# tooHotSpot/FGN

Measured on AMD Instinct MI355X. Metric: query-imgs/sec (3-way 3-shot, 800x1333 FGN simple_test), higher is better.
Workload: dtype f32; 1 GPU; cfg3: COCO2VOC 3-way 3-shot, query 3x800x1333, supports 9x3x256^2, ResNet-50-C4, R<=300 proposals, D<=100 detections, 1 episode(s) per GPU per step; h2d_in_step=True, gt_mask_rle_in_step=True, world_size_seen=1, phase_lock=rpn, caller_streams=2, support_cache=False, hip_graph=True, winograd_3x3=F(4x4,3x3)

## Files before the change

fgn_amd/csrc/conv_igemm.hip:

```cpp
#include "common.h"
#include <cstdlib>

struct ConvParams {
    const float* x;
    const float* w;
    float* y;
    const float* scale;
    const float* shift;
    const float* residual;
    const float* in_scale;
    const int32_t* n_img_dev;
    int n_img, H, W, Cin, Ho, Wo, Cout, KH, KW, stride, pad;
    int a_img_div;
    int relu;
    int K;
    int n_tiles_n;
    int band_nt, band_mt;
    float* ws;
    int splits, kt_per_split;
#ifdef FGN_EXPERIMENTS
    int32_t* tickets;
    int32_t* sched;
    int sk_U, sk_dp;
#endif
// ... 1378 lines not shown
                                            const void* w_x3, float* y, const float* shift, int rows, int Cin1, int Cin2,
                                            int Cout, int cout_pad, int relu, hipStream_t stream) {
    if (!x || !x2 || !w_x3 || !y) return FGN_ERR_ARG;
    if (rows <= 0) return FGN_OK;
    if (Cin1 % BK || Cin2 % BK || Cin1 <= 0 || Cin2 <= 0 || (Cout & 3) || cout_pad % X3_BN || cout_pad < Cout) return FGN_ERR_SHAPE;
    if ((!x2_rows && x2_total_rows != rows) || x2_total_rows < 1) return FGN_ERR_ARG;
    const int K = Cin1 + Cin2;
    const long long xb = (long long)rows * Cin1 * 4, x2b = (long long)x2_total_rows * Cin2 * 4;
    const long long wb = (long long)fgn_x3_image_bytes(K, cout_pad, 1);
    if (xb >= 0x7fffff00ll || x2b >= 0x7fffff00ll || wb >= 0x7fffff00ll || (long long)rows * Cout >= (1ll << 31)) return FGN_ERR_SHAPE;
    ConvParams p;
    x3_base_params(p);
    p.x = x; p.y = y; p.shift = shift;
    p.x2 = x2; p.x2_bytes = (unsigned)x2b; p.kt1 = Cin1 / BK; p.cin2 = Cin2; p.x2_rows = x2_rows;
    p.n_img = rows; p.Cin = Cin1; p.Cout = Cout; p.relu = relu; p.K = K;
    p.kt_per_split = K / BK; p.x_bytes = (unsigned)xb;
    p.w3 = w_x3; p.w3_bytes = (unsigned)wb; p.npad3 = cout_pad;
    return launch_x3(p, rows, 0, 6, stream);
}

extern "C" int fgn_winograd_gemm_x3_f32(const float* V, const void* U_x3, float* Mo, const int32_t* n_img_dev, int n_img,
                                        int tiles_per_img, int t_pad, int Cin, int Cout, int cout_pad, int n_groups,
                                        hipStream_t stream) {
    if (!V || !U_x3 || !Mo) return FGN_ERR_ARG;
    if (n_img <= 0) return FGN_OK;
    if (Cin % BK != 0 || Cin < 2 * BK || Cout % 4 != 0 || cout_pad % X3_BN != 0 || cout_pad < Cout || t_pad % 64 != 0 ||
        (n_groups != 16 && n_groups != 36) || (long long)n_img * tiles_per_img > t_pad)
        return FGN_ERR_SHAPE;
    const long long rows = (long long)n_groups * t_pad;
    const long long xb = rows * Cin * 4, wb = (long long)fgn_x3_image_bytes(Cin, cout_pad, n_groups);
    if (xb >= 0x7fffff00ll || wb >= 0x7fffff00ll || rows * Cout >= (1ll << 31)) return FGN_ERR_SHAPE;
    ConvParams p;
    x3_base_params(p);
    p.x = V; p.y = Mo;
    p.n_img = (int)rows; p.Cin = Cin; p.Cout = Cout; p.K = Cin; p.kt_per_split = Cin / BK; p.x_bytes = (unsigned)xb;
    p.grp_rows = t_pad; p.grp_valid = n_img * tiles_per_img; p.grp_items = n_img;
    p.grp_rows_per_item = tiles_per_img; p.grp_count_dev = n_img_dev;
    p.w3 = U_x3; p.w3_bytes = (unsigned)wb; p.npad3 = cout_pad;
    return launch_x3(p, (int)rows, 0, 6, stream);
}

static int h2_pick(long long M, int Cout, int K, int grp_rows, int grp_valid, int bm) {
    if (bm == 264) return (grp_rows && grp_rows % 128) ? 0 : 264;
    if (bm != 0) return x3_pick_bm(M, Cout, K, grp_rows, grp_valid, bm);
    if (Cout <= 64) {
        if (grp_rows && grp_rows % 128) return 0;
        if (Cout < 48 || (M + 127) / 128 < 256) return 0;
        return 264;
    }
    const int bm_x3 = x3_pick_bm(M, Cout, K, grp_rows, grp_valid, 0);
    return (bm_x3 == 128 && !grp_rows) ? 64 : bm_x3;
}

template <int WMW, int WNW, int RB, int NST, bool IM2COL>
static int launch_h2_cfg(ConvParams& p, const H2Im2col& q2, int M_max, hipStream_t stream) {
    constexpr int BM = 32 * RB * WMW, BN = 64 * WNW;
    const int m_tiles = cdiv(M_max, BM);
    p.n_tiles_n = cdiv(p.Cout, BN);
    {
        const long long per_nt = (long long)BN * p.K * 4;
        p.band_nt = 0; p.band_mt = 0;
        if (per_nt * p.n_tiles_n > 2048 * 1024) {
            int nb = (int)std::max<long long>(1, 2048 * 1024 / per_nt);
            while (nb > 1 && p.n_tiles_n % nb) --nb;
            const int mt = p.grp_rows ? p.grp_rows / BM : m_tiles;
            if (nb < p.n_tiles_n && mt > 0 && m_tiles % mt == 0) { p.band_nt = nb; p.band_mt = mt; }
        }
    }
    const int tiles = m_tiles * p.n_tiles_n;
    static unsigned long long ok = 0ull;
    hipError_t attr = fgn_allow_full_lds(reinterpret_cast<const void*>(conv_pw_h2_kernel<WMW, WNW, RB, NST, IM2COL>), &ok);
    if (attr != hipSuccess) return (int)attr;
    const size_t lds = (size_t)NST * (BM * 128 + 2 * BN * 64);
    const int per_cu = std::min(3, (int)(160 * 1024 / lds));
    const int grid = std::min(256 * per_cu, (tiles + 7) / 8 * 8);
    p.stamp = fgn_next_stamp_record();
    FGN_LAUNCH_TIMED((conv_pw_h2_kernel<WMW, WNW, RB, NST, IM2COL>), dim3(grid), dim3(64 * WMW * WNW), lds, stream, p, q2, tiles);
    FGN_LAUNCH_CHECK();
    return FGN_OK;
}

extern "C" size_t fgn_h2_image_bytes(int K, int npad, int n_groups) { return (size_t)n_groups * npad * ((size_t)K * 4 + 4); }
extern "C" int fgn_h2_row_tile(long long M, int Cout, int K, int grp_rows, int grp_valid) {
    return h2_pick(M, Cout, K, grp_rows, grp_valid, 0);
}

static int launch_h2(const ConvParams& p0, int M_max, int n_groups, int bm, hipStream_t stream, const H2Im2col* im = nullptr) {
    ConvParams p = p0;
    if (!p.w3 || p.npad3 % H2_BN || p.npad3 < p.Cout || (p.Cout & 3) || p.K % BK || p.K < 2 * BK || p.splits != 1) return FGN_ERR_SHAPE;
    const size_t img = (size_t)n_groups * p.K * p.npad3 * 4;
    p.w3_bytes = (unsigned)img;
    p.w_inv = reinterpret_cast<const float*>(static_cast<const char*>(p.w3) + img);
    H2Im2col none;
    none.y1 = nullptr; none.x_off0 = none.x_off1 = 0u; none.M0 = none.M1 = 0; none.H1 = none.W1 = none.Ho1 = none.Wo1 = 1; none.cin_shift = 0;
    if (bm != 0 && bm != 64 && bm != 128 && bm != 264) return FGN_ERR_SHAPE;
    const int cfg = h2_pick(M_max, p.Cout, p.K, p.grp_rows, p.grp_valid, bm);
    if (cfg == 0) return FGN_ERR_SHAPE;
    if (im) {
        if (cfg == 264) return launch_h2_cfg<4, 1, 1, 2, true>(p, *im, M_max, stream);
        return cfg == 128 ? launch_h2_cfg<2, 2, 2, 2, true>(p, *im, M_max, stream) : launch_h2_cfg<2, 2, 1, 2, true>(p, *im, M_max, stream);
    }
    if (cfg == 264) return launch_h2_cfg<4, 1, 1, 2, false>(p, none, M_max, stream);
    return cfg == 128 ? launch_h2_cfg<2, 2, 2, 2, false>(p, none, M_max, stream) : launch_h2_cfg<2, 2, 1, 2, false>(p, none, M_max, stream);
}

extern "C" int fgn_conv2d_pair_h2_nhwc_f32(const float* x0, int n_img0, int H0, int W0, const float* x1, int n_img1, int H1,
                                           int W1, const void* w_h2, float* y0, float* y1, const float* scale,
                                           const float* shift, int Cin, int Cout, int cout_pad, int KH, int KW, int stride,
                                           int pad, int relu, hipStream_t stream) {
    if (!x0 || !w_h2 || !y0 || (x1 && !y1)) return FGN_ERR_ARG;
    if (n_img0 <= 0 || (x1 && n_img1 <= 0)) return FGN_ERR_SHAPE;
    const int ct = Cin / BK;
    if (Cin % BK || (ct & (ct - 1)) || KH != KW || (KW != 1 && KW != 3) || stride < 1 || pad < 0 || (Cout & 3) ||
        cout_pad % H2_BN || cout_pad < Cout || H0 <= 0 || W0 <= 0)
        return FGN_ERR_SHAPE;
    const int Ho0 = (H0 + 2 * pad - KH) / stride + 1, Wo0 = (W0 + 2 * pad - KW) / stride + 1;
    const int Ho1 = x1 ? (H1 + 2 * pad - KH) / stride + 1 : 1, Wo1 = x1 ? (W1 + 2 * pad - KW) / stride + 1 : 1;
    if (Ho0 <= 0 || Wo0 <= 0 || Ho1 <= 0 || Wo1 <= 0) return FGN_ERR_SHAPE;
    const long long M0 = (long long)n_img0 * Ho0 * Wo0, M1 = x1 ? (long long)n_img1 * Ho1 * Wo1 : 0;
    const long long b0 = (long long)n_img0 * H0 * W0 * Cin * 4, b1 = x1 ? (long long)n_img1 * H1 * W1 * Cin * 4 : 0;
    const char* lo = reinterpret_cast<const char*>(x0);
    if (x1 && reinterpret_cast<const char*>(x1) < lo) lo = reinterpret_cast<const char*>(x1);
    const long long off0 = reinterpret_cast<const char*>(x0) - lo, off1 = x1 ? reinterpret_cast<const char*>(x1) - lo : 0;
    const long long span = std::max(off0 + b0, off1 + b1);
    const int K = KH * KW * Cin;
    const long long wb = (long long)fgn_h2_image_bytes(K, cout_pad, 1);
    if (span >= 0x7fffff00ll || wb >= 0x7fffff00ll || (M0 + M1) * Cout >= (1ll << 31)) return FGN_ERR_SHAPE;
    ConvParams p;
    x3_base_params(p);
    p.x = reinterpret_cast<const float*>(lo); p.x_bytes = (unsigned)span; p.y = y0; p.scale = scale; p.shift = shift;
    p.n_img = n_img0; p.H = H0; p.W = W0; p.Ho = Ho0; p.Wo = Wo0; p.Cin = Cin; p.Cout = Cout; p.relu = relu;
    p.KH = KH; p.KW = KW; p.stride = stride; p.pad = pad; p.K = K; p.kt_per_split = K / BK;
    p.w3 = w_h2; p.npad3 = cout_pad;
    H2Im2col q;
    q.y1 = y1; q.x_off0 = (unsigned)off0; q.x_off1 = (unsigned)off1; q.M0 = (int)M0; q.M1 = (int)M1;
    q.H1 = x1 ? H1 : 1; q.W1 = x1 ? W1 : 1; q.Ho1 = Ho1; q.Wo1 = Wo1;
    q.cin_shift = 0;
    while ((1 << q.cin_shift) < ct) ++q.cin_shift;
    return launch_h2(p, (int)(M0 + M1), 1, 0, stream, &q);
}

extern "C" int fgn_gemm_h2_f32(const float* x, const void* w_h2, float* y, const float* shift, const float* residual,
                               int rows, int K, int Cout, int npad, int relu, int grp_rows, int grp_valid, int n_groups,
                               int bm, hipStream_t stream) {
    if (!x || !w_h2 || !y) return FGN_ERR_ARG;
    if (rows <= 0) return FGN_OK;
    if (K % BK || K <= 0 || (Cout & 3) || npad % H2_BN || npad < Cout || n_groups < 1) return FGN_ERR_SHAPE;
    if (n_groups > 1 && (grp_rows <= 0 || (long long)n_groups * grp_rows != rows || grp_valid > grp_rows)) return FGN_ERR_SHAPE;
    const long long xb = (long long)rows * K * 4, wb = (long long)fgn_h2_image_bytes(K, npad, n_groups);
    if (xb >= 0x7fffff00ll || wb >= 0x7fffff00ll || (long long)rows * Cout >= (1ll << 31)) return FGN_ERR_SHAPE;
    ConvParams p;
    x3_base_params(p);
    p.x = x; p.y = y; p.shift = shift; p.residual = residual;
    p.n_img = rows; p.Cin = K; p.Cout = Cout; p.relu = relu; p.K = K; p.kt_per_split = K / BK; p.x_bytes = (unsigned)xb;
    p.grp_rows = n_groups > 1 ? grp_rows : 0; p.grp_valid = grp_valid;
    p.w3 = w_h2; p.npad3 = npad;
// ... 98 lines not shown
```

fgn_amd/csrc/conv_pw_h2.h:

```cpp
#pragma once

typedef _Float16 f16x8_t __attribute__((ext_vector_type(8)));

struct H2Frag { f16x8_t hi, lo; };

__device__ __forceinline__ void h2_split4(const float x0, const float x1, const float x2, const float x3, const float s,
                                          unsigned& h01, unsigned& h23, unsigned& l01, unsigned& l23) {
    asm("v_fma_mixlo_f16 %0, %4, %8, 0\n\t"
        "v_fma_mixlo_f16 %1, %6, %8, 0\n\t"
        "v_fma_mixhi_f16 %0, %5, %8, 0\n\t"
        "v_fma_mixhi_f16 %1, %7, %8, 0\n\t"
        "v_fma_mixlo_f16 %2, %4, %8, -%0 op_sel:[0,0,0] op_sel_hi:[0,0,1]\n\t"
        "v_fma_mixlo_f16 %3, %6, %8, -%1 op_sel:[0,0,0] op_sel_hi:[0,0,1]\n\t"
        "v_fma_mixhi_f16 %2, %5, %8, -%0 op_sel:[0,0,1] op_sel_hi:[0,0,1]\n\t"
        "v_fma_mixhi_f16 %3, %7, %8, -%1 op_sel:[0,0,1] op_sel_hi:[0,0,1]\n\t"
        "s_nop 1"
        : "=&v"(h01), "=&v"(h23), "=&v"(l01), "=&v"(l23)
        : "v"(x0), "v"(x1), "v"(x2), "v"(x3), "s"(s));
}

__device__ __forceinline__ H2Frag h2_split(const float4& a, const float4& b, const float s) {
    unsigned h[4], l[4];
    h2_split4(a.x, a.y, a.z, a.w, s, h[0], h[1], l[0], l[1]);
    h2_split4(b.x, b.y, b.z, b.w, s, h[2], h[3], l[2], l[3]);
    H2Frag f;
    f.hi = __builtin_bit_cast(f16x8_t, make_uint4(h[0], h[1], h[2], h[3]));
    f.lo = __builtin_bit_cast(f16x8_t, make_uint4(l[0], l[1], l[2], l[3]));
    return f;
}

__device__ __forceinline__ float h2_absmax16(const float4& a, const float4& b, const float4& c, const float4& d) {
    float m;
    asm("v_max3_f32 %0, |%1|, |%2|, 0\n\t"
        "v_max3_f32 %0, |%3|, |%4|, %0\n\t"
        "v_max3_f32 %0, |%5|, |%6|, %0\n\t"
        "v_max3_f32 %0, |%7|, |%8|, %0\n\t"
        "v_max3_f32 %0, |%9|, |%10|, %0\n\t"
        "v_max3_f32 %0, |%11|, |%12|, %0\n\t"
        "v_max3_f32 %0, |%13|, |%14|, %0\n\t"
        "v_max3_f32 %0, |%15|, |%16|, %0"
        : "=&v"(m)
        : "v"(a.x), "v"(a.y), "v"(a.z), "v"(a.w), "v"(b.x), "v"(b.y), "v"(b.z), "v"(b.w),
          "v"(c.x), "v"(c.y), "v"(c.z), "v"(c.w), "v"(d.x), "v"(d.y), "v"(d.z), "v"(d.w));
    return m;
}

constexpr int H2_BN = 128;

struct H2Im2col {
    float* y1;
    unsigned x_off0, x_off1;
    int M0, M1;
    int H1, W1, Ho1, Wo1;
    int cin_shift;
};

template <int WMW, int WNW, int RB, int NST, bool IM2COL>
__global__ __launch_bounds__(64 * WMW * WNW, 2) void conv_pw_h2_kernel(const ConvParams p, const H2Im2col q2, const int total_tiles) {
    constexpr int BM = 32 * RB * WMW, BN = 64 * WNW, NTHR = 64 * WMW * WNW, NW = WMW * WNW;
    constexpr int A_LD = BM / 8 / NW;
    constexpr int A_STAGE = BM * 128;
    constexpr int B_STAGE = 2 * BN * 64;
    constexpr int STAGE = A_STAGE + B_STAGE;
    constexpr int BQ = BN / 16;
    constexpr int B_LD = 2 * BQ / NW;
    static_assert(A_LD * 8 * NW == BM && B_LD * NW == 2 * BQ, "tile / wave split");
    constexpr int PER = A_LD + B_LD;
    constexpr int D = NST - 1;
    constexpr int ROWS_PER_PASS = NTHR / 8;
    static_assert(NST == 2 || NST == 3, "ring of 2 or 3 stages");
    extern __shared__ __attribute__((aligned(16))) unsigned char smem_h2[];

    const int t = threadIdx.x, lane = t & 63, wv = t >> 6;
    const int wm = wv / WNW, wn = wv % WNW;
    const int M = IM2COL ? q2.M0 + q2.M1 : (p.n_img_dev ? min(p.n_img, *p.n_img_dev) : p.n_img) * p.Ho * p.Wo;
    int grp_valid = p.grp_valid;
    if (p.grp_rows && p.grp_count_dev) grp_valid = min(grp_valid, min(p.grp_items, *p.grp_count_dev) * p.grp_rows_per_item);

    float a_s = 1.f, a_inv = 1.f;

    const int col4 = t & 7, row0 = t >> 3;
    const int src_c4 = col4 ^ ((row0 >> 1) & 7);
    const i32x4 x_rs = make_rsrc(p.x, p.x_bytes);
    const i32x4 w_rs = make_rsrc(p.w3, p.w3_bytes);
    const bool dual = !IM2COL && p.x2 != nullptr;
    const i32x4 x2_rs = make_rsrc(dual ? p.x2 : p.x, dual ? p.x2_bytes : p.x_bytes);
    const int KT = p.K / BK;
    const unsigned kt_bytes = (unsigned)(2 * p.npad3 * 64);
    const unsigned lds_base = __builtin_amdgcn_readfirstlane((unsigned)reinterpret_cast<size_t>(smem_h2));
    const unsigned wave_row_bytes = __builtin_amdgcn_readfirstlane(wv) * 8 * 128;
    constexpr unsigned OOB = 0x7ffffff0u;

    const int nq = total_tiles >> 3, nr = total_tiles & 7;
    auto coords = [&](int tile, int& m0, int& n0) -> bool {
        const int xcd = tile & 7, idx = tile >> 3;
        const int bid = (xcd < nr ? xcd * (nq + 1) : nr * (nq + 1) + (xcd - nr) * nq) + idx;
        int tile_m = bid / p.n_tiles_n;
        int tile_n = bid - tile_m * p.n_tiles_n;
        if (p.band_nt > 0) {
            const int per_grp = p.band_mt * p.n_tiles_n;
            const int grp = bid / per_grp;
            int r = bid - grp * per_grp;
            const int per_band = p.band_mt * p.band_nt;
            const int band = r / per_band;
            r -= band * per_band;
            const int mi = r / p.band_nt;
            tile_m = grp * p.band_mt + mi;
            tile_n = band * p.band_nt + (r - mi * p.band_nt);
        }
        m0 = tile_m * BM;
        n0 = tile_n * BN;
        if (m0 >= M) return false;
// ... 39 lines not shown
                        for (int kx = 0; kx < p.KW; ++kx, ++tp)
                            if (y_ok && (unsigned)(ix0 + kx) < (unsigned)W) tm |= 1u << tp;
                    }
                    o.a2[i] = tm;
                }
                continue;
            }
            const bool in = m < M && m < g_end;
            o.a[i] = in ? (unsigned)((m * p.Cin + src_c4 * 4) * 4) : OOB;
            o.a2[i] = OOB;
            if (dual && in) o.a2[i] = (unsigned)(((p.x2_rows ? p.x2_rows[m] : m) * p.cin2 + src_c4 * 4) * 4);
        }
        unsigned g0 = 0;
        if (p.grp_rows) g0 = (unsigned)(m0 / p.grp_rows) * (unsigned)KT * kt_bytes;
#pragma unroll
        for (int i = 0; i < B_LD; ++i) {
            const int q = wv + NW * i;
            const int plane = q / BQ, row = (q % BQ) * 16 + (lane >> 2);
            o.b[i] = g0 + (unsigned)(((plane * p.npad3 + n0 + row) * 4 + (lane & 3)) * 16);
        }
        return o;
    };
    auto issue = [&](const Offs& o, int kt, int stage) {
        const unsigned st = lds_base + stage * STAGE;
        const unsigned sa = st + wave_row_bytes;
        const unsigned ko = (unsigned)(kt * BK * 4);
        if constexpr (IM2COL) {
            const int tap = kt >> q2.cin_shift;
            const int c0 = (kt - (tap << q2.cin_shift)) * BK;
            const int ky = p.KW == 3 ? (tap * 43) >> 7 : tap;
            const int kx = tap - ky * p.KW;
            const unsigned off0 = (unsigned)(((ky * p.W + kx) * p.Cin + c0) * 4);
            const unsigned off1 = (unsigned)(((ky * q2.W1 + kx) * p.Cin + c0) * 4);
#pragma unroll
            for (int i = 0; i < A_LD; ++i) {
                const bool ok = (o.a2[i] >> tap) & 1u;
                const unsigned voff = ok ? o.a[i] + ((o.a2[i] >> 31) ? off1 : off0) : OOB;
                lds_dma16_s(x_rs, sa + i * ROWS_PER_PASS * 128, voff, 0u);
            }
        } else if (dual && kt >= p.kt1) {
            const unsigned ko2 = (unsigned)((kt - p.kt1) * BK * 4);
#pragma unroll
            for (int i = 0; i < A_LD; ++i) lds_dma16_s(x2_rs, sa + i * ROWS_PER_PASS * 128, o.a2[i], ko2);
        } else {
#pragma unroll
            for (int i = 0; i < A_LD; ++i) lds_dma16_s(x_rs, sa + i * ROWS_PER_PASS * 128, o.a[i], ko);
        }
        const unsigned kb = (unsigned)kt * kt_bytes;
#pragma unroll
        for (int i = 0; i < B_LD; ++i) lds_dma16_s(w_rs, st + b_lds[i], o.b[i], kb);
    };

    const int r16 = lane & 15, g4 = lane >> 4;
    const int a16_row = wm * 32 * RB + r16;
    const unsigned a16_sw = (unsigned)((a16_row >> 1) & 7);
    const unsigned a16_rd0 = (unsigned)(a16_row * 128) + ((((unsigned)g4) ^ a16_sw) << 4);
    const unsigned a16_rd1 = (unsigned)(a16_row * 128) + ((((unsigned)(g4 + 4)) ^ a16_sw) << 4);
    const int n16 = wn * 64 + r16;
    const unsigned tau16 = (0x1230u >> (4 * ((n16 >> 2) & 3))) & 3u;
    const unsigned b16_rd = (unsigned)(A_STAGE + n16 * 64) + ((((unsigned)g4) ^ tau16) << 4);

    if (p.stamp && t == 0 && blockIdx.x == 0) atomicExch(p.stamp, __builtin_amdgcn_s_memrealtime());
    auto leave = [&]() {
        if (!p.stamp || t != 0) return;
        const unsigned shard = blockIdx.x & 7u;
        const unsigned long long in_shard = (gridDim.x - shard + 7u) / 8u;
        unsigned long long* const sc = p.stamp + 8 * (1 + shard);
        if (atomicAdd(sc, 1ull) != in_shard - 1) return;
        atomicExch(sc, 0ull);
        const unsigned long long shards = gridDim.x < 8u ? gridDim.x : 8u;
        if (atomicAdd(p.stamp + 2, 1ull) != shards - 1) return;
        const unsigned long long d = __builtin_amdgcn_s_memrealtime() - atomicExch(p.stamp, 0ull);
        atomicExch(p.stamp + 2, 0ull);
        atomicAdd(p.stamp + 1, d);
        atomicAdd(p.stamp + 3, 1ull);
        atomicMin(p.stamp + 4, d);
        atomicMax(p.stamp + 5, d);
    };

    int m0, n0, nm0 = 0, nn0 = 0;
    int tile = next_active(blockIdx.x, m0, n0);
    if (tile < 0) { leave(); return; }
    Offs cur = offsets(m0, n0);
    int ntile = next_active(tile + gridDim.x, nm0, nn0);
    Offs nxt = cur;
    if (ntile >= 0) nxt = offsets(nm0, nn0);
    int ic_kt = 0, ic_stage = 0, ahead = 0;
    bool ic_next = false;
    auto issue_one = [&]() {
        if (!ic_next) {
            issue(cur, ic_kt, ic_stage);
            if (++ic_kt == KT) { ic_next = true; ic_kt = 0; }
        } else {
            if (ntile < 0 || ic_kt >= KT) return;
            issue(nxt, ic_kt, ic_stage);
            ++ic_kt;
        }
        ic_stage = ic_stage + 1 == NST ? 0 : ic_stage + 1;
        ++ahead;
    };
#pragma unroll
    for (int i = 0; i < D; ++i) issue_one();
    int stage = 0;

    while (true) {
        f32x4 acc[2 * RB][4];
#pragma unroll
        for (int i = 0; i < 2 * RB; ++i)
#pragma unroll
            for (int j = 0; j < 4; ++j) acc[i][j] = f32x4{0.f, 0.f, 0.f, 0.f};
        bool have_s = false;
        float a_lim = 0.f;
        a_s = 1.f; a_inv = 1.f;
        for (int kt = 0; kt < KT; ++kt) {
            if (D == 2 && kt > 0 && ahead == 2) x3_wait_vm<PER>(); else x3_wait_vm<0>();
            asm volatile("s_waitcnt lgkmcnt(0)" ::: "memory");
            __builtin_amdgcn_s_barrier();
            --ahead;
            issue_one();
            asm volatile("" ::: "memory");
            const unsigned char* const S = smem_h2 + stage * STAGE;
            float4 alo[2 * RB], ahi[2 * RB];
            f16x8_t bq[4][2];
#pragma unroll
            for (int i = 0; i < 2 * RB; ++i) {
                alo[i] = *reinterpret_cast<const float4*>(S + a16_rd0 + i * (16 * 128));
                ahi[i] = *reinterpret_cast<const float4*>(S + a16_rd1 + i * (16 * 128));
            }
#pragma unroll
            for (int j = 0; j < 4; ++j)
#pragma unroll
                for (int q = 0; q < 2; ++q)
                    bq[j][q] = *reinterpret_cast<const f16x8_t*>(S + b16_rd + j * (16 * 64) + q * (BN * 64));
            __builtin_amdgcn_sched_barrier(0);
            auto adapt = [&]() {
                float m = 0.f;
#pragma unroll
                for (int i = 0; i < 2 * RB; ++i) {
                    m = fmaxf(m, fmaxf(fmaxf(fabsf(alo[i].x), fabsf(alo[i].y)), fmaxf(fabsf(alo[i].z), fabsf(alo[i].w))));
                    m = fmaxf(m, fmaxf(fmaxf(fabsf(ahi[i].x), fabsf(ahi[i].y)), fmaxf(fabsf(ahi[i].z), fabsf(ahi[i].w))));
                }
#pragma unroll
                for (int o = 32; o > 0; o >>= 1) m = fmaxf(m, __shfl_xor(m, o));
                const unsigned mb = __builtin_amdgcn_readfirstlane(__float_as_uint(m));
                const int e = (int)((mb >> 23) & 0xffu);
                if (e < 27 || e == 255) return;
                const float ns = __uint_as_float((unsigned)(267 - e) << 23);
                const float ratio = ns * a_inv;
                if (have_s) {
#pragma unroll
                    for (int i = 0; i < 2 * RB; ++i)
#pragma unroll
                        for (int j = 0; j < 4; ++j) acc[i][j] *= ratio;
                }
                a_s = ns;
                a_inv = __uint_as_float((unsigned)(e - 13) << 23);
                a_lim = 65504.f * a_inv;
                have_s = true;
            };
            {
                float big = h2_absmax16(alo[0], ahi[0], alo[1], ahi[1]);
                if constexpr (RB == 2) big = fmaxf(big, h2_absmax16(alo[2], ahi[2], alo[3], ahi[3]));
                if (__builtin_expect(__builtin_amdgcn_ballot_w64(!(big <= a_lim)) != 0ull, 0)) adapt();
            }
#pragma unroll
            for (int i = 0; i < 2 * RB; ++i) {
                const H2Frag a = h2_split(alo[i], ahi[i], a_s);
#pragma unroll
                for (int j = 0; j < 4; ++j) {
                    f32x4 c = acc[i][j];
                    c = __builtin_amdgcn_mfma_f32_16x16x32_f16(a.lo, bq[j][0], c, 0, 0, 0);
                    c = __builtin_amdgcn_mfma_f32_16x16x32_f16(a.hi, bq[j][1], c, 0, 0, 0);
                    c = __builtin_amdgcn_mfma_f32_16x16x32_f16(a.hi, bq[j][0], c, 0, 0, 0);
                    acc[i][j] = c;
                }
            }
            stage = stage + 1 == NST ? 0 : stage + 1;
        }
        float* const cbase = reinterpret_cast<float*>(smem_h2 + (stage == 0 ? NST - 1 : stage - 1) * STAGE);
        const int em0 = m0, en0 = n0;
        const float* const winv = p.w_inv + (p.grp_rows ? (size_t)(em0 / p.grp_rows) * p.npad3 : 0);
        constexpr int PR = 32 * RB;
#pragma unroll
        for (int pass = 0; pass < WMW; ++pass) {
            __syncthreads();
            if (wm == pass) {
#pragma unroll
                for (int i = 0; i < 2 * RB; ++i)
#pragma unroll
                    for (int j = 0; j < 4; ++j) {
                        float* cw = cbase + (16 * i + 4 * g4) * BN + wn * 64 + 16 * j + r16;
#pragma unroll
                        for (int r = 0; r < 4; ++r) cw[r * BN] = acc[i][j][r] * a_inv;
                    }
            }
            __syncthreads();
            constexpr int C4 = BN / 4, RPP = NTHR / C4, NPASS = PR / RPP, SW = NPASS < 4 ? NPASS : 4;
            static_assert(NPASS % SW == 0, "row sweeps in groups of SW");
            const int c4 = t % C4, rr = t / C4;
            const int n = en0 + c4 * 4;
            if (n < p.Cout) {
                float4 sc = make_float4(1.f, 1.f, 1.f, 1.f), sh = make_float4(0.f, 0.f, 0.f, 0.f);
                if (p.scale) sc = *reinterpret_cast<const float4*>(p.scale + n);
                if (p.shift) sh = *reinterpret_cast<const float4*>(p.shift + n);
                const float4 iv = *reinterpret_cast<const float4*>(winv + n);
#pragma unroll
                for (int k0 = 0; k0 < NPASS; k0 += SW) {
                    float4 res[SW];
#pragma unroll
                    for (int k = 0; k < SW; ++k) {
                        const int m = em0 + PR * pass + rr + RPP * (k0 + k);
                        res[k] = make_float4(0.f, 0.f, 0.f, 0.f);
                        if (p.residual && m < M) res[k] = *reinterpret_cast<const float4*>(p.residual + (size_t)m * p.Cout + n);
                    }
#pragma unroll
                    for (int k = 0; k < SW; ++k) {
                        const int row = rr + RPP * (k0 + k);
                        const int m = em0 + PR * pass + row;
                        if (m >= M) continue;
                        float4 v = *reinterpret_cast<const float4*>(cbase + row * BN + c4 * 4);
                        v.x *= iv.x; v.y *= iv.y; v.z *= iv.z; v.w *= iv.w;
                        v.x = v.x * sc.x + sh.x; v.y = v.y * sc.y + sh.y; v.z = v.z * sc.z + sh.z; v.w = v.w * sc.w + sh.w;
                        v.x += res[k].x; v.y += res[k].y; v.z += res[k].z; v.w += res[k].w;
                        if (p.relu) {
                            v.x = fmaxf(v.x, 0.f); v.y = fmaxf(v.y, 0.f); v.z = fmaxf(v.z, 0.f); v.w = fmaxf(v.w, 0.f);
                        }
                        float* const yrow = (IM2COL && m >= q2.M0) ? q2.y1 + (size_t)(m - q2.M0) * p.Cout : p.y + (size_t)m * p.Cout;
                        *reinterpret_cast<float4*>(yrow + n) = v;
                    }
                }
            }
        }
        if (ntile < 0) break;
        tile = ntile; m0 = nm0; n0 = nn0;
        cur = nxt;
        ic_next = ic_kt >= KT;
        if (ic_next) ic_kt = 0;
        ntile = next_active(tile + gridDim.x, nm0, nn0);
        if (ntile >= 0) nxt = offsets(nm0, nn0);
    }
    asm volatile("s_waitcnt vmcnt(0)" ::: "memory");
    leave();
}
```

fgn_amd/ops.py:

```python
from __future__ import annotations

import ctypes as C
import math
import os
from dataclasses import dataclass
from typing import Optional

import numpy as np
import torch

from . import lib as _lib


PROFILE = None

FUSED_SHORTCUT = os.environ.get('FGN_FUSED_SHORTCUT', '1') != '0'
GEMM_MATH = os.environ.get('FGN_GEMM_MATH', 'h2')
X3_KERNELS = {64: 'conv_pw_x3_kernel<2, 1, 6, 2, true>', 128: 'conv_pw_x3_kernel<2, 2, 6, 2, true>'}
H2_KERNELS = {64: 'conv_pw_h2_kernel<2, 2, 1, 2, %s>', 128: 'conv_pw_h2_kernel<2, 2, 2, 2, %s>', 264: 'conv_pw_h2_kernel<4, 1, 1, 2, %s>'}


def x3_kernel(rows: int, cout: int, k: int, grp_rows: int = 0, grp_valid: int = 0) -> str:
    return X3_KERNELS.get(_lib.load().fgn_x3_row_tile(rows, cout, k, grp_rows, grp_valid), 'conv_pw_x3_kernel<?>')


def h2_kernel(rows: int, cout: int, k: int, grp_rows: int = 0, grp_valid: int = 0, im2col: bool = False) -> str:
    return H2_KERNELS.get(_lib.load().fgn_h2_row_tile(rows, cout, k, grp_rows, grp_valid), 'conv_pw_h2_kernel<?, %s>') % ('true' if im2col else 'false')


class gemm_math:

    def __init__(self, mode):
        self.mode = mode

    def __enter__(self):
        global GEMM_MATH
        self.prev = GEMM_MATH
        if self.mode is not None:
            GEMM_MATH = self.mode
        return self

    def __exit__(self, *exc):
        global GEMM_MATH
        GEMM_MATH = self.prev
        return False
FUSED_SHORTCUT_STRIDES = tuple(int(v) for v in os.environ.get('FGN_FUSED_SHORTCUT_STRIDES', '1,2').split(','))

_TILES = {1: (128, 128, 64, 64, 2), 2: (64, 128, 32, 64, 3), 3: (128, 64, 64, 32, 3), 4: (64, 64, 32, 32, 4)}


def kernel_name(kid: int) -> str:
    mode = kid % 10
    bm, bn, wm, wn, mw = _TILES[kid // 10]
    if mode == 4:
        return 'conv_pw_persist_kernel'
    if mode == 3:
        return f'conv_igemm_kernel<{bm}, {bn}, {wm}, {wn}, *, {mw}>'
    return f'conv_igemm_dma_kernel<{bm}, {bn}, {wm}, {wn}, 2, {mw}, {mode}>'


class ZeroArena:

    def __init__(self, device, nbytes: int = 2 << 20):
        self.buf = torch.zeros(nbytes, dtype=torch.uint8, device=device)
        self.off = 0

    def take(self, shape, dtype):
        n = int(np.prod(shape)) * torch.empty((), dtype=dtype).element_size()
        start = (self.off + 255) // 256 * 256
        if start + n > self.buf.numel():
            return None
        self.off = start + n
# ... 1508 lines not shown
```

Baseline: 319.4 img/s.

## Generalize h2 GEMM wave tile to MB x NB and switch to 4x1 wave layouts

New measurement: 322.1 img/s, median of 6. Within noise of the previous version (+0.8%).

```diff
diff --git a/fgn_amd/csrc/conv_igemm.hip b/fgn_amd/csrc/conv_igemm.hip
--- a/fgn_amd/csrc/conv_igemm.hip
+++ b/fgn_amd/csrc/conv_igemm.hip
@@ -1454,9 +1454,9 @@
     return (bm_x3 == 128 && !grp_rows) ? 64 : bm_x3;
 }
 
-template <int WMW, int WNW, int RB, int NST, bool IM2COL>
+template <int WMW, int WNW, int MB, int NB, int NST, bool IM2COL>
 static int launch_h2_cfg(ConvParams& p, const H2Im2col& q2, int M_max, hipStream_t stream) {
-    constexpr int BM = 32 * RB * WMW, BN = 64 * WNW;
+    constexpr int BM = 16 * MB * WMW, BN = 16 * NB * WNW;
     const int m_tiles = cdiv(M_max, BM);
     p.n_tiles_n = cdiv(p.Cout, BN);
     {
@@ -1471,13 +1471,13 @@
     }
     const int tiles = m_tiles * p.n_tiles_n;
     static unsigned long long ok = 0ull;
-    hipError_t attr = fgn_allow_full_lds(reinterpret_cast<const void*>(conv_pw_h2_kernel<WMW, WNW, RB, NST, IM2COL>), &ok);
+    hipError_t attr = fgn_allow_full_lds(reinterpret_cast<const void*>(conv_pw_h2_kernel<WMW, WNW, MB, NB, NST, IM2COL>), &ok);
     if (attr != hipSuccess) return (int)attr;
     const size_t lds = (size_t)NST * (BM * 128 + 2 * BN * 64);
     const int per_cu = std::min(3, (int)(160 * 1024 / lds));
     const int grid = std::min(256 * per_cu, (tiles + 7) / 8 * 8);
     p.stamp = fgn_next_stamp_record();
-    FGN_LAUNCH_TIMED((conv_pw_h2_kernel<WMW, WNW, RB, NST, IM2COL>), dim3(grid), dim3(64 * WMW * WNW), lds, stream, p, q2, tiles);
+    FGN_LAUNCH_TIMED((conv_pw_h2_kernel<WMW, WNW, MB, NB, NST, IM2COL>), dim3(grid), dim3(64 * WMW * WNW), lds, stream, p, q2, tiles);
     FGN_LAUNCH_CHECK();
     return FGN_OK;
 }
@@ -1499,11 +1499,11 @@
     const int cfg = h2_pick(M_max, p.Cout, p.K, p.grp_rows, p.grp_valid, bm);
     if (cfg == 0) return FGN_ERR_SHAPE;
     if (im) {
-        if (cfg == 264) return launch_h2_cfg<4, 1, 1, 2, true>(p, *im, M_max, stream);
-        return cfg == 128 ? launch_h2_cfg<2, 2, 2, 2, true>(p, *im, M_max, stream) : launch_h2_cfg<2, 2, 1, 2, true>(p, *im, M_max, stream);
-    }
-    if (cfg == 264) return launch_h2_cfg<4, 1, 1, 2, false>(p, none, M_max, stream);
-    return cfg == 128 ? launch_h2_cfg<2, 2, 2, 2, false>(p, none, M_max, stream) : launch_h2_cfg<2, 2, 1, 2, false>(p, none, M_max, stream);
+        if (cfg == 264) return launch_h2_cfg<4, 1, 2, 4, 2, true>(p, *im, M_max, stream);
+        return cfg == 128 ? launch_h2_cfg<4, 1, 2, 8, 2, true>(p, *im, M_max, stream) : launch_h2_cfg<4, 1, 1, 8, 2, true>(p, *im, M_max, stream);
+    }
+    if (cfg == 264) return launch_h2_cfg<4, 1, 2, 4, 2, false>(p, none, M_max, stream);
+    return cfg == 128 ? launch_h2_cfg<4, 1, 2, 8, 2, false>(p, none, M_max, stream) : launch_h2_cfg<4, 1, 1, 8, 2, false>(p, none, M_max, stream);
 }
 
 extern "C" int fgn_conv2d_pair_h2_nhwc_f32(const float* x0, int n_img0, int H0, int W0, const float* x1, int n_img1, int H1,
diff --git a/fgn_amd/csrc/conv_pw_h2.h b/fgn_amd/csrc/conv_pw_h2.h
--- a/fgn_amd/csrc/conv_pw_h2.h
+++ b/fgn_amd/csrc/conv_pw_h2.h
@@ -27,6 +27,17 @@
     f.hi = __builtin_bit_cast(f16x8_t, make_uint4(h[0], h[1], h[2], h[3]));
     f.lo = __builtin_bit_cast(f16x8_t, make_uint4(l[0], l[1], l[2], l[3]));
     return f;
+}
+
+__device__ __forceinline__ float h2_absmax8(const float4& a, const float4& b) {
+    float m;
+    asm("v_max3_f32 %0, |%1|, |%2|, 0\n\t"
+        "v_max3_f32 %0, |%3|, |%4|, %0\n\t"
+        "v_max3_f32 %0, |%5|, |%6|, %0\n\t"
+        "v_max3_f32 %0, |%7|, |%8|, %0"
+        : "=&v"(m)
+        : "v"(a.x), "v"(a.y), "v"(a.z), "v"(a.w), "v"(b.x), "v"(b.y), "v"(b.z), "v"(b.w));
+    return m;
 }
 
 __device__ __forceinline__ float h2_absmax16(const float4& a, const float4& b, const float4& c, const float4& d) {
@@ -55,9 +66,10 @@
     int cin_shift;
 };
 
-template <int WMW, int WNW, int RB, int NST, bool IM2COL>
+template <int WMW, int WNW, int MB, int NB, int NST, bool IM2COL>
 __global__ __launch_bounds__(64 * WMW * WNW, 2) void conv_pw_h2_kernel(const ConvParams p, const H2Im2col q2, const int total_tiles) {
-    constexpr int BM = 32 * RB * WMW, BN = 64 * WNW, NTHR = 64 * WMW * WNW, NW = WMW * WNW;
+    constexpr int BM = 16 * MB * WMW, BN = 16 * NB * WNW, NTHR = 64 * WMW * WNW, NW = WMW * WNW;
+    static_assert((MB == 1 || MB == 2 || MB == 4) && (NB == 4 || NB == 8), "wave tile");
     constexpr int A_LD = BM / 8 / NW;
     constexpr int A_STAGE = BM * 128;
     constexpr int B_STAGE = 2 * BN * 64;
@@ -203,11 +215,11 @@
     };
 
     const int r16 = lane & 15, g4 = lane >> 4;
-    const int a16_row = wm * 32 * RB + r16;
+    const int a16_row = wm * 16 * MB + r16;
     const unsigned a16_sw = (unsigned)((a16_row >> 1) & 7);
     const unsigned a16_rd0 = (unsigned)(a16_row * 128) + ((((unsigned)g4) ^ a16_sw) << 4);
     const unsigned a16_rd1 = (unsigned)(a16_row * 128) + ((((unsigned)(g4 + 4)) ^ a16_sw) << 4);
-    const int n16 = wn * 64 + r16;
+    const int n16 = wn * 16 * NB + r16;
     const unsigned tau16 = (0x1230u >> (4 * ((n16 >> 2) & 3))) & 3u;
     const unsigned b16_rd = (unsigned)(A_STAGE + n16 * 64) + ((((unsigned)g4) ^ tau16) << 4);
 
@@ -255,11 +267,11 @@
     int stage = 0;
 
     while (true) {
-        f32x4 acc[2 * RB][4];
-#pragma unroll
-        for (int i = 0; i < 2 * RB; ++i)
-#pragma unroll
-            for (int j = 0; j < 4; ++j) acc[i][j] = f32x4{0.f, 0.f, 0.f, 0.f};
+        f32x4 acc[MB][NB];
+#pragma unroll
+        for (int i = 0; i < MB; ++i)
+#pragma unroll
+            for (int j = 0; j < NB; ++j) acc[i][j] = f32x4{0.f, 0.f, 0.f, 0.f};
         bool have_s = false;
         float a_lim = 0.f;
         a_s = 1.f; a_inv = 1.f;
@@ -271,15 +283,15 @@
             issue_one();
             asm volatile("" ::: "memory");
             const unsigned char* const S = smem_h2 + stage * STAGE;
-            float4 alo[2 * RB], ahi[2 * RB];
-            f16x8_t bq[4][2];
-#pragma unroll
-            for (int i = 0; i < 2 * RB; ++i) {
+            float4 alo[MB], ahi[MB];
+            f16x8_t bq[NB][2];
+#pragma unroll
+            for (int i = 0; i < MB; ++i) {
                 alo[i] = *reinterpret_cast<const float4*>(S + a16_rd0 + i * (16 * 128));
                 ahi[i] = *reinterpret_cast<const float4*>(S + a16_rd1 + i * (16 * 128));
             }
 #pragma unroll
-            for (int j = 0; j < 4; ++j)
+            for (int j = 0; j < NB; ++j)
 #pragma unroll
                 for (int q = 0; q < 2; ++q)
                     bq[j][q] = *reinterpret_cast<const f16x8_t*>(S + b16_rd + j * (16 * 64) + q * (BN * 64));
@@ -287,7 +299,7 @@
             auto adapt = [&]() {
                 float m = 0.f;
 #pragma unroll
-                for (int i = 0; i < 2 * RB; ++i) {
+                for (int i = 0; i < MB; ++i) {
                     m = fmaxf(m, fmaxf(fmaxf(fabsf(alo[i].x), fabsf(alo[i].y)), fmaxf(fabsf(alo[i].z), fabsf(alo[i].w))));
                     m = fmaxf(m, fmaxf(fmaxf(fabsf(ahi[i].x), fabsf(ahi[i].y)), fmaxf(fabsf(ahi[i].z), fabsf(ahi[i].w))));
                 }
@@ -300,9 +312,9 @@
                 const float ratio = ns * a_inv;
                 if (have_s) {
 #pragma unroll
-                    for (int i = 0; i < 2 * RB; ++i)
-#pragma unroll
-                        for (int j = 0; j < 4; ++j) acc[i][j] *= ratio;
+                    for (int i = 0; i < MB; ++i)
+#pragma unroll
+                        for (int j = 0; j < NB; ++j) acc[i][j] *= ratio;
                 }
                 a_s = ns;
                 a_inv = __uint_as_float((unsigned)(e - 13) << 23);
@@ -310,15 +322,17 @@
                 have_s = true;
             };
             {
-                float big = h2_absmax16(alo[0], ahi[0], alo[1], ahi[1]);
-                if constexpr (RB == 2) big = fmaxf(big, h2_absmax16(alo[2], ahi[2], alo[3], ahi[3]));
+                float big;
+                if constexpr (MB == 1) big = h2_absmax8(alo[0], ahi[0]);
+                else big = h2_absmax16(alo[0], ahi[0], alo[1], ahi[1]);
+                if constexpr (MB == 4) big = fmaxf(big, h2_absmax16(alo[2], ahi[2], alo[3], ahi[3]));
                 if (__builtin_expect(__builtin_amdgcn_ballot_w64(!(big <= a_lim)) != 0ull, 0)) adapt();
             }
 #pragma unroll
-            for (int i = 0; i < 2 * RB; ++i) {
+            for (int i = 0; i < MB; ++i) {
                 const H2Frag a = h2_split(alo[i], ahi[i], a_s);
 #pragma unroll
-                for (int j = 0; j < 4; ++j) {
+                for (int j = 0; j < NB; ++j) {
                     f32x4 c = acc[i][j];
                     c = __builtin_amdgcn_mfma_f32_16x16x32_f16(a.lo, bq[j][0], c, 0, 0, 0);
                     c = __builtin_amdgcn_mfma_f32_16x16x32_f16(a.hi, bq[j][1], c, 0, 0, 0);
@@ -331,22 +345,24 @@
         float* const cbase = reinterpret_cast<float*>(smem_h2 + (stage == 0 ? NST - 1 : stage - 1) * STAGE);
         const int em0 = m0, en0 = n0;
         const float* const winv = p.w_inv + (p.grp_rows ? (size_t)(em0 / p.grp_rows) * p.npad3 : 0);
-        constexpr int PR = 32 * RB;
-#pragma unroll
-        for (int pass = 0; pass < WMW; ++pass) {
+        constexpr int PR = 16 * MB;
+        constexpr int WPP = (BN == H2_BN && WMW % 2 == 0 && 2 * PR * BN * 4 <= STAGE) ? 2 : 1;
+        static_assert(WPP * PR * BN * 4 <= STAGE, "C tile pass fits the stage");
+#pragma unroll
+        for (int pass = 0; pass < WMW / WPP; ++pass) {
             __syncthreads();
-            if (wm == pass) {
-#pragma unroll
-                for (int i = 0; i < 2 * RB; ++i)
-#pragma unroll
-                    for (int j = 0; j < 4; ++j) {
-                        float* cw = cbase + (16 * i + 4 * g4) * BN + wn * 64 + 16 * j + r16;
+            if (wm / WPP == pass) {
+#pragma unroll
+                for (int i = 0; i < MB; ++i)
+#pragma unroll
+                    for (int j = 0; j < NB; ++j) {
+                        float* cw = cbase + ((wm % WPP) * PR + 16 * i + 4 * g4) * BN + wn * 16 * NB + 16 * j + r16;
 #pragma unroll
                         for (int r = 0; r < 4; ++r) cw[r * BN] = acc[i][j][r] * a_inv;
                     }
             }
             __syncthreads();
-            constexpr int C4 = BN / 4, RPP = NTHR / C4, NPASS = PR / RPP, SW = NPASS < 4 ? NPASS : 4;
+            constexpr int C4 = BN / 4, RPP = NTHR / C4, NPASS = WPP * PR / RPP, SW = NPASS < 4 ? NPASS : 4;
             static_assert(NPASS % SW == 0, "row sweeps in groups of SW");
             const int c4 = t % C4, rr = t / C4;
             const int n = en0 + c4 * 4;
@@ -360,14 +376,14 @@
                     float4 res[SW];
 #pragma unroll
                     for (int k = 0; k < SW; ++k) {
-                        const int m = em0 + PR * pass + rr + RPP * (k0 + k);
+                        const int m = em0 + WPP * PR * pass + rr + RPP * (k0 + k);
                         res[k] = make_float4(0.f, 0.f, 0.f, 0.f);
                         if (p.residual && m < M) res[k] = *reinterpret_cast<const float4*>(p.residual + (size_t)m * p.Cout + n);
                     }
 #pragma unroll
                     for (int k = 0; k < SW; ++k) {
                         const int row = rr + RPP * (k0 + k);
-                        const int m = em0 + PR * pass + row;
+                        const int m = em0 + WPP * PR * pass + row;
                         if (m >= M) continue;
                         float4 v = *reinterpret_cast<const float4*>(cbase + row * BN + c4 * 4);
                         v.x *= iv.x; v.y *= iv.y; v.z *= iv.z; v.w *= iv.w;
diff --git a/fgn_amd/ops.py b/fgn_amd/ops.py
--- a/fgn_amd/ops.py
+++ b/fgn_amd/ops.py
@@ -17,7 +17,7 @@
 FUSED_SHORTCUT = os.environ.get('FGN_FUSED_SHORTCUT', '1') != '0'
 GEMM_MATH = os.environ.get('FGN_GEMM_MATH', 'h2')
 X3_KERNELS = {64: 'conv_pw_x3_kernel<2, 1, 6, 2, true>', 128: 'conv_pw_x3_kernel<2, 2, 6, 2, true>'}
-H2_KERNELS = {64: 'conv_pw_h2_kernel<2, 2, 1, 2, %s>', 128: 'conv_pw_h2_kernel<2, 2, 2, 2, %s>', 264: 'conv_pw_h2_kernel<4, 1, 1, 2, %s>'}
+H2_KERNELS = {64: 'conv_pw_h2_kernel<4, 1, 1, 8, 2, %s>', 128: 'conv_pw_h2_kernel<4, 1, 2, 8, 2, %s>', 264: 'conv_pw_h2_kernel<4, 1, 2, 4, 2, %s>'}
 
 
 def x3_kernel(rows: int, cout: int, k: int, grp_rows: int = 0, grp_valid: int = 0) -> str:
```

## Generalize h2 GEMM warp tiling and switch to 4x1 wave layouts

Applied to the files above, without the earlier changes.

Result: no change. 322.0 img/s before, 323.4 img/s after (median of 6 runs) (+0.5%).

```diff
diff --git a/fgn_amd/csrc/conv_igemm.hip b/fgn_amd/csrc/conv_igemm.hip
--- a/fgn_amd/csrc/conv_igemm.hip
+++ b/fgn_amd/csrc/conv_igemm.hip
@@ -1454,9 +1454,9 @@
     return (bm_x3 == 128 && !grp_rows) ? 64 : bm_x3;
 }
 
-template <int WMW, int WNW, int RB, int NST, bool IM2COL>
+template <int WMW, int WNW, int MB, int NB, int NST, bool IM2COL>
 static int launch_h2_cfg(ConvParams& p, const H2Im2col& q2, int M_max, hipStream_t stream) {
-    constexpr int BM = 32 * RB * WMW, BN = 64 * WNW;
+    constexpr int BM = 16 * MB * WMW, BN = 16 * NB * WNW;
     const int m_tiles = cdiv(M_max, BM);
     p.n_tiles_n = cdiv(p.Cout, BN);
     {
@@ -1471,13 +1471,13 @@
     }
     const int tiles = m_tiles * p.n_tiles_n;
     static unsigned long long ok = 0ull;
-    hipError_t attr = fgn_allow_full_lds(reinterpret_cast<const void*>(conv_pw_h2_kernel<WMW, WNW, RB, NST, IM2COL>), &ok);
+    hipError_t attr = fgn_allow_full_lds(reinterpret_cast<const void*>(conv_pw_h2_kernel<WMW, WNW, MB, NB, NST, IM2COL>), &ok);
     if (attr != hipSuccess) return (int)attr;
     const size_t lds = (size_t)NST * (BM * 128 + 2 * BN * 64);
     const int per_cu = std::min(3, (int)(160 * 1024 / lds));
     const int grid = std::min(256 * per_cu, (tiles + 7) / 8 * 8);
     p.stamp = fgn_next_stamp_record();
-    FGN_LAUNCH_TIMED((conv_pw_h2_kernel<WMW, WNW, RB, NST, IM2COL>), dim3(grid), dim3(64 * WMW * WNW), lds, stream, p, q2, tiles);
+    FGN_LAUNCH_TIMED((conv_pw_h2_kernel<WMW, WNW, MB, NB, NST, IM2COL>), dim3(grid), dim3(64 * WMW * WNW), lds, stream, p, q2, tiles);
     FGN_LAUNCH_CHECK();
     return FGN_OK;
 }
@@ -1499,11 +1499,11 @@
     const int cfg = h2_pick(M_max, p.Cout, p.K, p.grp_rows, p.grp_valid, bm);
     if (cfg == 0) return FGN_ERR_SHAPE;
     if (im) {
-        if (cfg == 264) return launch_h2_cfg<4, 1, 1, 2, true>(p, *im, M_max, stream);
-        return cfg == 128 ? launch_h2_cfg<2, 2, 2, 2, true>(p, *im, M_max, stream) : launch_h2_cfg<2, 2, 1, 2, true>(p, *im, M_max, stream);
-    }
-    if (cfg == 264) return launch_h2_cfg<4, 1, 1, 2, false>(p, none, M_max, stream);
-    return cfg == 128 ? launch_h2_cfg<2, 2, 2, 2, false>(p, none, M_max, stream) : launch_h2_cfg<2, 2, 1, 2, false>(p, none, M_max, stream);
+        if (cfg == 264) return launch_h2_cfg<4, 1, 2, 4, 2, true>(p, *im, M_max, stream);
+        return cfg == 128 ? launch_h2_cfg<4, 1, 2, 8, 2, true>(p, *im, M_max, stream) : launch_h2_cfg<4, 1, 1, 8, 2, true>(p, *im, M_max, stream);
+    }
+    if (cfg == 264) return launch_h2_cfg<4, 1, 2, 4, 2, false>(p, none, M_max, stream);
+    return cfg == 128 ? launch_h2_cfg<4, 1, 2, 8, 2, false>(p, none, M_max, stream) : launch_h2_cfg<4, 1, 1, 8, 2, false>(p, none, M_max, stream);
 }
 
 extern "C" int fgn_conv2d_pair_h2_nhwc_f32(const float* x0, int n_img0, int H0, int W0, const float* x1, int n_img1, int H1,
diff --git a/fgn_amd/csrc/conv_pw_h2.h b/fgn_amd/csrc/conv_pw_h2.h
--- a/fgn_amd/csrc/conv_pw_h2.h
+++ b/fgn_amd/csrc/conv_pw_h2.h
@@ -27,6 +27,17 @@
     f.hi = __builtin_bit_cast(f16x8_t, make_uint4(h[0], h[1], h[2], h[3]));
     f.lo = __builtin_bit_cast(f16x8_t, make_uint4(l[0], l[1], l[2], l[3]));
     return f;
+}
+
+__device__ __forceinline__ float h2_absmax8(const float4& a, const float4& b) {
+    float m;
+    asm("v_max3_f32 %0, |%1|, |%2|, 0\n\t"
+        "v_max3_f32 %0, |%3|, |%4|, %0\n\t"
+        "v_max3_f32 %0, |%5|, |%6|, %0\n\t"
+        "v_max3_f32 %0, |%7|, |%8|, %0"
+        : "=&v"(m)
+        : "v"(a.x), "v"(a.y), "v"(a.z), "v"(a.w), "v"(b.x), "v"(b.y), "v"(b.z), "v"(b.w));
+    return m;
 }
 
 __device__ __forceinline__ float h2_absmax16(const float4& a, const float4& b, const float4& c, const float4& d) {
@@ -55,9 +66,9 @@
     int cin_shift;
 };
 
-template <int WMW, int WNW, int RB, int NST, bool IM2COL>
+template <int WMW, int WNW, int MB, int NB, int NST, bool IM2COL>
 __global__ __launch_bounds__(64 * WMW * WNW, 2) void conv_pw_h2_kernel(const ConvParams p, const H2Im2col q2, const int total_tiles) {
-    constexpr int BM = 32 * RB * WMW, BN = 64 * WNW, NTHR = 64 * WMW * WNW, NW = WMW * WNW;
+    constexpr int BM = 16 * MB * WMW, BN = 16 * NB * WNW, NTHR = 64 * WMW * WNW, NW = WMW * WNW;
     constexpr int A_LD = BM / 8 / NW;
     constexpr int A_STAGE = BM * 128;
     constexpr int B_STAGE = 2 * BN * 64;
@@ -203,11 +214,11 @@
     };
 
     const int r16 = lane & 15, g4 = lane >> 4;
-    const int a16_row = wm * 32 * RB + r16;
+    const int a16_row = wm * 16 * MB + r16;
     const unsigned a16_sw = (unsigned)((a16_row >> 1) & 7);
     const unsigned a16_rd0 = (unsigned)(a16_row * 128) + ((((unsigned)g4) ^ a16_sw) << 4);
     const unsigned a16_rd1 = (unsigned)(a16_row * 128) + ((((unsigned)(g4 + 4)) ^ a16_sw) << 4);
-    const int n16 = wn * 64 + r16;
+    const int n16 = wn * 16 * NB + r16;
     const unsigned tau16 = (0x1230u >> (4 * ((n16 >> 2) & 3))) & 3u;
     const unsigned b16_rd = (unsigned)(A_STAGE + n16 * 64) + ((((unsigned)g4) ^ tau16) << 4);
 
@@ -255,11 +266,11 @@
     int stage = 0;
 
     while (true) {
-        f32x4 acc[2 * RB][4];
-#pragma unroll
-        for (int i = 0; i < 2 * RB; ++i)
-#pragma unroll
-            for (int j = 0; j < 4; ++j) acc[i][j] = f32x4{0.f, 0.f, 0.f, 0.f};
+        f32x4 acc[MB][NB];
+#pragma unroll
+        for (int i = 0; i < MB; ++i)
+#pragma unroll
+            for (int j = 0; j < NB; ++j) acc[i][j] = f32x4{0.f, 0.f, 0.f, 0.f};
         bool have_s = false;
         float a_lim = 0.f;
         a_s = 1.f; a_inv = 1.f;
@@ -271,38 +282,39 @@
             issue_one();
             asm volatile("" ::: "memory");
             const unsigned char* const S = smem_h2 + stage * STAGE;
-            float4 alo[2 * RB], ahi[2 * RB];
-            f16x8_t bq[4][2];
-#pragma unroll
-            for (int i = 0; i < 2 * RB; ++i) {
+            float4 alo[MB], ahi[MB];
+            f16x8_t bq[NB][2];
+#pragma unroll
+            for (int i = 0; i < MB; ++i) {
                 alo[i] = *reinterpret_cast<const float4*>(S + a16_rd0 + i * (16 * 128));
                 ahi[i] = *reinterpret_cast<const float4*>(S + a16_rd1 + i * (16 * 128));
             }
 #pragma unroll
-            for (int j = 0; j < 4; ++j)
+            for (int j = 0; j < NB; ++j)
 #pragma unroll
                 for (int q = 0; q < 2; ++q)
                     bq[j][q] = *reinterpret_cast<const f16x8_t*>(S + b16_rd + j * (16 * 64) + q * (BN * 64));
             __builtin_amdgcn_sched_barrier(0);
             auto adapt = [&]() {
+                auto fin = [](float x) { x = fabsf(x); return x < __builtin_huge_valf() ? x : 0.f; };
                 float m = 0.f;
 #pragma unroll
-                for (int i = 0; i < 2 * RB; ++i) {
-                    m = fmaxf(m, fmaxf(fmaxf(fabsf(alo[i].x), fabsf(alo[i].y)), fmaxf(fabsf(alo[i].z), fabsf(alo[i].w))));
-                    m = fmaxf(m, fmaxf(fmaxf(fabsf(ahi[i].x), fabsf(ahi[i].y)), fmaxf(fabsf(ahi[i].z), fabsf(ahi[i].w))));
+                for (int i = 0; i < MB; ++i) {
+                    m = fmaxf(m, fmaxf(fmaxf(fin(alo[i].x), fin(alo[i].y)), fmaxf(fin(alo[i].z), fin(alo[i].w))));
+                    m = fmaxf(m, fmaxf(fmaxf(fin(ahi[i].x), fin(ahi[i].y)), fmaxf(fin(ahi[i].z), fin(ahi[i].w))));
                 }
 #pragma unroll
                 for (int o = 32; o > 0; o >>= 1) m = fmaxf(m, __shfl_xor(m, o));
                 const unsigned mb = __builtin_amdgcn_readfirstlane(__float_as_uint(m));
                 const int e = (int)((mb >> 23) & 0xffu);
-                if (e < 27 || e == 255) return;
+                if (e < 27) return;
                 const float ns = __uint_as_float((unsigned)(267 - e) << 23);
                 const float ratio = ns * a_inv;
                 if (have_s) {
 #pragma unroll
-                    for (int i = 0; i < 2 * RB; ++i)
-#pragma unroll
-                        for (int j = 0; j < 4; ++j) acc[i][j] *= ratio;
+                    for (int i = 0; i < MB; ++i)
+#pragma unroll
+                        for (int j = 0; j < NB; ++j) acc[i][j] *= ratio;
                 }
                 a_s = ns;
                 a_inv = __uint_as_float((unsigned)(e - 13) << 23);
@@ -310,15 +322,17 @@
                 have_s = true;
             };
             {
-                float big = h2_absmax16(alo[0], ahi[0], alo[1], ahi[1]);
-                if constexpr (RB == 2) big = fmaxf(big, h2_absmax16(alo[2], ahi[2], alo[3], ahi[3]));
+                float big;
+                if constexpr (MB == 1) big = h2_absmax8(alo[0], ahi[0]);
+                else big = h2_absmax16(alo[0], ahi[0], alo[1], ahi[1]);
+                if constexpr (MB == 4) big = fmaxf(big, h2_absmax16(alo[2], ahi[2], alo[3], ahi[3]));
                 if (__builtin_expect(__builtin_amdgcn_ballot_w64(!(big <= a_lim)) != 0ull, 0)) adapt();
             }
 #pragma unroll
-            for (int i = 0; i < 2 * RB; ++i) {
+            for (int i = 0; i < MB; ++i) {
                 const H2Frag a = h2_split(alo[i], ahi[i], a_s);
 #pragma unroll
-                for (int j = 0; j < 4; ++j) {
+                for (int j = 0; j < NB; ++j) {
                     f32x4 c = acc[i][j];
                     c = __builtin_amdgcn_mfma_f32_16x16x32_f16(a.lo, bq[j][0], c, 0, 0, 0);
                     c = __builtin_amdgcn_mfma_f32_16x16x32_f16(a.hi, bq[j][1], c, 0, 0, 0);
@@ -331,16 +345,19 @@
         float* const cbase = reinterpret_cast<float*>(smem_h2 + (stage == 0 ? NST - 1 : stage - 1) * STAGE);
         const int em0 = m0, en0 = n0;
         const float* const winv = p.w_inv + (p.grp_rows ? (size_t)(em0 / p.grp_rows) * p.npad3 : 0);
-        constexpr int PR = 32 * RB;
-#pragma unroll
-        for (int pass = 0; pass < WMW; ++pass) {
+        constexpr int WROW = 16 * MB * BN * 4;
+        constexpr int WPP = (WMW >= 4 && 4 * WROW <= STAGE) ? 4 : (WMW >= 2 && 2 * WROW <= STAGE) ? 2 : 1;
+        static_assert(WMW % WPP == 0 && WPP * WROW <= STAGE, "C tile passes");
+        constexpr int PR = 16 * MB * WPP;
+#pragma unroll
+        for (int pass = 0; pass < WMW / WPP; ++pass) {
             __syncthreads();
-            if (wm == pass) {
-#pragma unroll
-                for (int i = 0; i < 2 * RB; ++i)
-#pragma unroll
-                    for (int j = 0; j < 4; ++j) {
-                        float* cw = cbase + (16 * i + 4 * g4) * BN + wn * 64 + 16 * j + r16;
+            if (wm / WPP == pass) {
+#pragma unroll
+                for (int i = 0; i < MB; ++i)
+#pragma unroll
+                    for (int j = 0; j < NB; ++j) {
+                        float* cw = cbase + (16 * MB * (wm % WPP) + 16 * i + 4 * g4) * BN + wn * 16 * NB + 16 * j + r16;
 #pragma unroll
                         for (int r = 0; r < 4; ++r) cw[r * BN] = acc[i][j][r] * a_inv;
                     }
diff --git a/fgn_amd/ops.py b/fgn_amd/ops.py
--- a/fgn_amd/ops.py
+++ b/fgn_amd/ops.py
@@ -17,7 +17,7 @@
 FUSED_SHORTCUT = os.environ.get('FGN_FUSED_SHORTCUT', '1') != '0'
 GEMM_MATH = os.environ.get('FGN_GEMM_MATH', 'h2')
 X3_KERNELS = {64: 'conv_pw_x3_kernel<2, 1, 6, 2, true>', 128: 'conv_pw_x3_kernel<2, 2, 6, 2, true>'}
-H2_KERNELS = {64: 'conv_pw_h2_kernel<2, 2, 1, 2, %s>', 128: 'conv_pw_h2_kernel<2, 2, 2, 2, %s>', 264: 'conv_pw_h2_kernel<4, 1, 1, 2, %s>'}
+H2_KERNELS = {64: 'conv_pw_h2_kernel<4, 1, 1, 8, 2, %s>', 128: 'conv_pw_h2_kernel<4, 1, 2, 8, 2, %s>', 264: 'conv_pw_h2_kernel<4, 1, 2, 4, 2, %s>'}
 
 
 def x3_kernel(rows: int, cout: int, k: int, grp_rows: int = 0, grp_valid: int = 0) -> str:
```
